# chenzpstar/Multi-Modal-Image-Fusion

Measured on AMD Instinct MI355X. Metric: image-pairs/sec at 256x256, PFNet train step, higher is better.
Workload: dtype bf16; 1 GPU; PFNetv1 train step (fwd + SSIM/pixel/grad losses + bwd + clip + Adam), 256x256 synthetic IR/visible pairs, batch 32 per GPU, bf16 feature maps / fp32 accumulate, random-init weights (seed 0); global_batch=32, parallelism=single

## Files before the change

### include/mmif.h

```cpp
#ifndef MMIF_H
#define MMIF_H

#include <stddef.h>
#include <stdint.h>

#ifdef __cplusplus
extern "C" {
#endif

#define MMIF_F32 0
#define MMIF_BF16 1

#define MMIF_IMPL_AUTO 0
#define MMIF_IMPL_VALU 1
#define MMIF_IMPL_MFMA 2
#define MMIF_IMPL_X3 3

#define MMIF_OK 0
#define MMIF_EINVAL (-1)
#define MMIF_ELAUNCH (-2)
#define MMIF_EWORKSPACE (-3)

typedef struct mmif_tensor {
    void* data;
// ... 242 lines not shown
size_t mmif_fusion_loss_workspace(int32_t n, int32_t h, int32_t w);
int mmif_fusion_loss(const float* img1, const float* img2, const float* imgf, int32_t n, int32_t h, int32_t w, float w_ssim,
                     float data_range, float w_pixel, int32_t pixel_max, int32_t pixel_l2, float w_grad, int32_t grad_max,
                     int32_t grad_l2, float* loss_out, float* grad_out, void* workspace, size_t workspace_bytes, void* stream);

int mmif_conv2d_bwd_pair_supported(int32_t cin, int32_t cout, int32_t ksize);
int mmif_conv2d_reflect_bwd_pair(const mmif_tensor* gy, const void* w_packed_t, const mmif_tensor* x, const mmif_tensor* gx, float* dw, float* db,
                                 int32_t cin, int32_t cout, int32_t ksize, int32_t accumulate, void* workspace, size_t workspace_bytes,
                                 void* stream);

int mmif_conv2d_bwd_wide_supported(int32_t cin, int32_t cout, int32_t ksize);
int mmif_conv2d_bwd_wide_supported_f32(int32_t cin, int32_t cout, int32_t ksize);
size_t mmif_conv2d_bwd_wide_signs_bytes(int32_t n, int32_t cin, int32_t h, int32_t w);
int mmif_conv2d_reflect_bwd_wide(const mmif_tensor* gy, const void* w_packed_t, const mmif_tensor* x, const mmif_tensor* gx, float* dw, float* db,
                                 int32_t cin, int32_t cout, int32_t ksize, uint64_t mask_bits, int32_t accumulate, void* workspace,
                                 size_t workspace_bytes, void* signs, size_t signs_bytes, void* stream);

typedef struct mmif_dense_encoder {
    const float* img;
    const float* w0;
    const float* b0;
    const void* packed[3];
    const float* bias[3];
} mmif_dense_encoder;
int mmif_dense_encoder_fwd(const mmif_dense_encoder* enc_a, const mmif_tensor* out_a, const mmif_dense_encoder* enc_b,
                           const mmif_tensor* out_b, void* stream);
int32_t mmif_dense_encoder_fwd_sum_supported(const mmif_dense_encoder* enc_a, const mmif_dense_encoder* enc_b, int32_t n, int32_t h, int32_t w);
int mmif_dense_encoder_fwd_sum(const mmif_dense_encoder* enc_a, const mmif_tensor* out_a, const mmif_dense_encoder* enc_b,
                               const mmif_tensor* out_b, const mmif_tensor* sum, void* stream);

size_t mmif_dense_encoder_wgrad_workspace(void);
int mmif_dense_encoder_wgrad(const float* img, const mmif_tensor* x, const mmif_tensor* gz, float* dw0, float* db0, float* dw1, float* db1,
                             float* dw2, float* db2, float* dw3, float* db3, int32_t accumulate, void* workspace, size_t workspace_bytes,
                             void* stream);

int mmif_pack_dense_chain(const float* w1, const float* w2, const float* w3, void* packed_v0, void* packed_v1, void* packed_v2,
                          void* stream);
int mmif_pack_dense_chain_pair(const float* const* w_a, void* const* packed_a, const float* const* w_b, void* const* packed_b, void* stream);
typedef struct mmif_dense_chain {
    const mmif_tensor* g3;
    const mmif_tensor* glow;
    const mmif_tensor* x;
    const void* packed[3];
    const mmif_tensor* out;
} mmif_dense_chain;
int mmif_dense_encoder_chain(const mmif_dense_chain* chain_a, const mmif_dense_chain* chain_b, void* stream);
int32_t mmif_dense_encoder_bwd_fits(int32_t cb_total, int32_t h, int32_t w, int32_t halo);
size_t mmif_dense_encoder_bwd_workspace(void);
int mmif_dense_encoder_bwd(const mmif_dense_chain* chain_a, const float* img_a, float* const* dwdb_a, int32_t accumulate_a,
                           const mmif_dense_chain* chain_b, const float* img_b, float* const* dwdb_b, int32_t accumulate_b,
                           void* workspace, size_t workspace_bytes, void* stream);
int mmif_pack_dense_chain_x3(const float* w1, const float* w2, const float* w3, void* packed_v0, void* packed_v1, void* packed_v2,
                             void* stream);

int mmif_patch_feed(const uint8_t* bank, int64_t n_patches, int32_t patch, const int32_t* idx, const int32_t* mode, int32_t batch,
                    int32_t norm_mode, float* out, void* stream);

size_t mmif_clip_adam_workspace(int64_t numel);
int mmif_clip_adam_step(float* params, const float* grads, float* exp_avg, float* exp_avg_sq, int64_t numel,
                        float lr, float beta1, float beta2, float eps, int32_t step, float max_norm,
                        float grad_scale, float* norm_out, void* workspace, size_t workspace_bytes, void* stream);

void mmif_debug_set_trace(void* device_buf);
void mmif_debug_set_conv_dma(int32_t mode);
void mmif_debug_set_conv1x1_stream(int32_t mode);
void mmif_debug_set_bwd_pair_dma(int32_t mode);
void mmif_debug_set_thin_wide(int32_t mode);
void mmif_debug_set_wgrad_dma_blocks(int32_t blocks);
void mmif_debug_set_ragged(int32_t mode);
int mmif_reduce_defer_begin(void* arena, size_t bytes);
int mmif_reduce_defer_flush(int32_t keep_deferring, void* stream);
int32_t mmif_reduce_defer_pending(void);

enum { MMIF_ROUTE_FWD = 0, MMIF_ROUTE_DGRAD = 1, MMIF_ROUTE_DGRAD_ONTO = 2, MMIF_ROUTE_DGRAD_DUP = 3, MMIF_ROUTE_WGRAD = 4, MMIF_ROUTE_BWD_PAIR = 5,
       MMIF_ROUTE_BWD_WIDE = 6 };
typedef struct {
    char name[32];
    int32_t G, slices, tiles, org;
} mmif_route;
int mmif_conv2d_route(int32_t op, const mmif_tensor* a, const mmif_tensor* b, int32_t cin, int32_t cout, int32_t ksize, uint64_t mask_bits,
                      uint64_t accum_bits, int32_t fold, int32_t impl, int32_t num_cus, mmif_route* out);

void mmif_debug_set_enc_stream2(int32_t mode);

#ifdef __cplusplus
}
#endif
#endif
```

### multi-modal-image-fusion_amd/csrc/loss.hip

```cpp
#include <math.h>

#include "common.hpp"

namespace mmif {

struct Win11 {
    float t[11];
};

constexpr int LT = 16;
constexpr int WIN = 11;

constexpr int ST = 32;
constexpr int SIN = ST + WIN - 1;
constexpr int SPI = 44;
constexpr int SPH = 36;

typedef float lf32x2 __attribute__((ext_vector_type(2)));

__device__ inline void ld16(const float* p, float (&v)[16]) {
#pragma unroll
    for (int i = 0; i < 4; ++i) {
        const float4 q = *reinterpret_cast<const float4*>(p + 4 * i);
        v[4 * i] = q.x; v[4 * i + 1] = q.y; v[4 * i + 2] = q.z; v[4 * i + 3] = q.w;
    }
}

__global__ __launch_bounds__(256, 2) void ssim_stats_kernel(const float* __restrict__ x1, const float* __restrict__ x2,
                                                            const float* __restrict__ f, int H, int W, Win11 win, float C1,
                                                            float C2, float* __restrict__ maps ,
                                                            float* __restrict__ partial, int tiles_x) {
    __shared__ __attribute__((aligned(16))) float in[3][SIN][SPI];
    __shared__ __attribute__((aligned(16))) float hb[8][SIN][SPH];
    __shared__ float red[16];
    const int Hm = H - WIN + 1, Wm = W - WIN + 1;
    const int tid = threadIdx.x;
    const int mx0 = (blockIdx.x % tiles_x) * ST, my0 = (blockIdx.x / tiles_x) * ST;
    const int in_ = blockIdx.y;
    const long long ibase = (long long)in_ * H * W;
    for (int e = tid; e < SIN * SPI; e += 256) {
        const int py = e / SPI, px = e % SPI;
        const int y = my0 + py, x = mx0 + px;
        const bool ok = (y < H) && (x < W) && px < SIN;
        const long long i = ibase + (long long)min(y, H - 1) * W + min(x, W - 1);
        const float a = x1[i], b = x2[i], c = f[i];
        in[0][py][px] = ok ? a : 0.f;
        in[1][py][px] = ok ? b : 0.f;
        in[2][py][px] = ok ? c : 0.f;
    }
    __syncthreads();
#pragma unroll 1
    for (int r = 0; r < 3; ++r) {
        const int it = tid + 256 * r, set = it / 384, idx = it - set * 384;
        if (idx >= SIN * 8) continue;
        const int py = idx >> 3, cg = idx & 7;
        float xa[16], fc[16];
        ld16(&in[set][py][4 * cg], xa);
        ld16(&in[2][py][4 * cg], fc);
        lf32x2 pa[14], pc[14];
#pragma unroll
        for (int i = 0; i < 14; ++i) {
            const float a = xa[i], c = fc[i];
            pa[i] = (lf32x2){a, a * a};
            pc[i] = (lf32x2){a * c, set ? c * c : c};
        }
        lf32x2 s01[4], s23[4];
#pragma unroll
        for (int j = 0; j < 4; ++j) s01[j] = s23[j] = (lf32x2){0.f, 0.f};
#pragma unroll
        for (int k = 0; k < WIN; ++k) {
            const lf32x2 wk = (lf32x2){win.t[k], win.t[k]};
#pragma unroll
            for (int j = 0; j < 4; ++j) {
                s01[j] = __builtin_elementwise_fma(wk, pa[j + k], s01[j]);
                s23[j] = __builtin_elementwise_fma(wk, pc[j + k], s23[j]);
            }
        }
        const int q0 = set ? 1 : 0, q1 = set ? 4 : 3, q2 = set ? 7 : 6, q3 = set ? 5 : 2;
        *reinterpret_cast<float4*>(&hb[q0][py][4 * cg]) = make_float4(s01[0].x, s01[1].x, s01[2].x, s01[3].x);
        *reinterpret_cast<float4*>(&hb[q1][py][4 * cg]) = make_float4(s01[0].y, s01[1].y, s01[2].y, s01[3].y);
        *reinterpret_cast<float4*>(&hb[q2][py][4 * cg]) = make_float4(s23[0].x, s23[1].x, s23[2].x, s23[3].x);
        *reinterpret_cast<float4*>(&hb[q3][py][4 * cg]) = make_float4(s23[0].y, s23[1].y, s23[2].y, s23[3].y);
    }
    __syncthreads();
    const int tx = tid & 31, rg = tid >> 5;
    float m[8][4];
#pragma unroll
    for (int q = 0; q < 8; q += 2) {
        lf32x2 v[14];
#pragma unroll
        for (int i = 0; i < 14; ++i) v[i] = (lf32x2){hb[q][4 * rg + i][tx], hb[q + 1][4 * rg + i][tx]};
#pragma unroll
        for (int j = 0; j < 4; ++j) {
            lf32x2 acc = (lf32x2){0.f, 0.f};
#pragma unroll
            for (int k = 0; k < WIN; ++k) acc = __builtin_elementwise_fma((lf32x2){win.t[k], win.t[k]}, v[j + k], acc);
            m[q][j] = acc.x;
            m[q + 1][j] = acc.y;
        }
    }
    float ssum = 0.f;
    const long long msz = (long long)gridDim.y * Hm * Wm;
#pragma unroll
    for (int j = 0; j < 4; ++j) {
        const int my = my0 + 4 * rg + j, mx = mx0 + tx;
        if (!((my < Hm) && (mx < Wm))) continue;
        const float mu1 = m[0][j], mu2 = m[1][j], muf = m[2][j];
        const float sf_raw = m[5][j] - muf * muf;
        const float sf = fmaxf(sf_raw, 0.f);
        const float kf = sf_raw > 0.f ? 1.f : 0.f;
        float A = 0.f, B = 0.f, Cs[2];
#pragma unroll
        for (int s2 = 0; s2 < 2; ++s2) {
            const float mux = s2 == 0 ? mu1 : mu2;
            const float ex2 = s2 == 0 ? m[3][j] : m[4][j];
            const float exf = s2 == 0 ? m[6][j] : m[7][j];
            const float sx = fmaxf(ex2 - mux * mux, 0.f);
            const float sxf = exf - mux * muf;
            const float m1 = 2.f * mux * muf + C1, m2 = mux * mux + muf * muf + C1;
            const float v1 = 2.f * sxf + C2, v2 = sx + sf + C2;
            const float inv = 1.f / (m2 * v2);
            const float S = m1 * v1 * inv;
            ssum += S;
            const float Bp = -(S / v2) * kf;
            const float Cp = 2.f * m1 * inv;
            const float Ap = 2.f * mux * v1 * inv - 2.f * muf * S / m2 - 2.f * mux * m1 * inv - 2.f * muf * Bp;
            A += Ap;
            B += Bp;
            Cs[s2] = Cp;
        }
        if (maps != nullptr) {
            const long long mi = ((long long)in_ * Hm + my) * Wm + mx;
            maps[mi] = A;
            maps[msz + mi] = B;
            maps[2 * msz + mi] = Cs[0];
            maps[3 * msz + mi] = Cs[1];
        }
    }
    const float bs = block_sum(ssum, red);
    if (tid == 0) partial[(long long)in_ * gridDim.x + blockIdx.x] = bs;
}

__global__ __launch_bounds__(256, 2) void ssim_grad_kernel(const float* __restrict__ x1, const float* __restrict__ x2,
                                                           const float* __restrict__ f, int H, int W, Win11 win,
                                                           const float* __restrict__ maps, float scale,
                                                           float* __restrict__ grad, int tiles_x) {
    __shared__ __attribute__((aligned(16))) float in[4][SIN][SPI];
    __shared__ __attribute__((aligned(16))) float hb[4][SIN][SPH];
    const int Hm = H - WIN + 1, Wm = W - WIN + 1;
    const int tid = threadIdx.x;
    const int x0 = (blockIdx.x % tiles_x) * ST, y0 = (blockIdx.x / tiles_x) * ST;
    const int in_ = blockIdx.y;
    const long long msz = (long long)gridDim.y * Hm * Wm;
    for (int e = tid; e < SIN * SPI; e += 256) {
        const int py = e / SPI, px = e % SPI;
        const int my = y0 - (WIN - 1) + py, mx = x0 - (WIN - 1) + px;
        const bool ok = my >= 0 && my < Hm && mx >= 0 && mx < Wm && px < SIN;
        const long long mi = ((long long)in_ * Hm + min(max(my, 0), Hm - 1)) * Wm + min(max(mx, 0), Wm - 1);
#pragma unroll
        for (int q = 0; q < 4; ++q) {
            const float v = maps[q * msz + mi];
            in[q][py][px] = ok ? v : 0.f;
        }
    }
    __syncthreads();
#pragma unroll 1
    for (int r = 0; r < 2; ++r) {
        const int idx = tid + 256 * r;
        if (idx >= SIN * 8) continue;
        const int py = idx >> 3, cg = idx & 7;
#pragma unroll
        for (int q = 0; q < 4; q += 2) {
            float v0[16], v1[16];
            ld16(&in[q][py][4 * cg], v0);
            ld16(&in[q + 1][py][4 * cg], v1);
            lf32x2 v[14];
#pragma unroll
            for (int i = 0; i < 14; ++i) v[i] = (lf32x2){v0[i], v1[i]};
            lf32x2 s2[4];
#pragma unroll
            for (int j = 0; j < 4; ++j) s2[j] = (lf32x2){0.f, 0.f};
#pragma unroll
            for (int k = 0; k < WIN; ++k)
#pragma unroll
                for (int j = 0; j < 4; ++j) s2[j] = __builtin_elementwise_fma((lf32x2){win.t[k], win.t[k]}, v[j + (WIN - 1) - k], s2[j]);
            *reinterpret_cast<float4*>(&hb[q][py][4 * cg]) = make_float4(s2[0].x, s2[1].x, s2[2].x, s2[3].x);
            *reinterpret_cast<float4*>(&hb[q + 1][py][4 * cg]) = make_float4(s2[0].y, s2[1].y, s2[2].y, s2[3].y);
        }
    }
    __syncthreads();
    const int tx = tid & 31, rg = tid >> 5;
    float m[4][4];
#pragma unroll
    for (int q = 0; q < 4; q += 2) {
        lf32x2 v[14];
#pragma unroll
        for (int i = 0; i < 14; ++i) v[i] = (lf32x2){hb[q][4 * rg + i][tx], hb[q + 1][4 * rg + i][tx]};
#pragma unroll
        for (int j = 0; j < 4; ++j) {
            lf32x2 acc = (lf32x2){0.f, 0.f};
#pragma unroll
            for (int k = 0; k < WIN; ++k) acc = __builtin_elementwise_fma((lf32x2){win.t[k], win.t[k]}, v[j + (WIN - 1) - k], acc);
            m[q][j] = acc.x;
            m[q + 1][j] = acc.y;
        }
    }
#pragma unroll
    for (int j = 0; j < 4; ++j) {
        const int y = y0 + 4 * rg + j, x = x0 + tx;
        if (y < H && x < W) {
            const long long i = ((long long)in_ * H + y) * W + x;
            grad[i] = scale * (m[0][j] + 2.f * f[i] * m[1][j] + x1[i] * m[2][j] + x2[i] * m[3][j]);
        }
    }
}

__global__ void ssim_finish_kernel(const float* __restrict__ partial, int np, float weight, float inv_count,
                                   float* __restrict__ loss) {
    __shared__ float red[16];
    float s = 0.f;
    for (int i = threadIdx.x; i < np; i += blockDim.x) s += partial[i];
    const float t = block_sum(s, red);
    if (threadIdx.x == 0) loss[0] = weight * (1.f - 0.5f * t * inv_count);
}

__global__ __launch_bounds__(256) void pixel_loss_kernel(const float* __restrict__ x1, const float* __restrict__ x2,
                                                         const float* __restrict__ f, long long total, float gscale,
                                                         int mode_max, int l2, float* __restrict__ grad,
                                                         float* __restrict__ partial, int accum) {
    __shared__ float red[16];
    float s = 0.f;
    for (long long i = (long long)blockIdx.x * blockDim.x + threadIdx.x; i < total; i += (long long)gridDim.x * blockDim.x) {
        const float a = x1[i], b = x2[i], c = f[i];
        float g;
        if (mode_max) {
            const float d = c - fmaxf(a, b);
            s += l2 ? d * d : fabsf(d);
            g = l2 ? 2.f * d : (d > 0.f ? 1.f : (d < 0.f ? -1.f : 0.f));
        } else {
            const float d1 = c - a, d2 = c - b;
            s += 0.5f * (l2 ? d1 * d1 + d2 * d2 : fabsf(d1) + fabsf(d2));
            g = 0.5f * (l2 ? 2.f * (d1 + d2)
                           : ((d1 > 0.f ? 1.f : (d1 < 0.f ? -1.f : 0.f)) + (d2 > 0.f ? 1.f : (d2 < 0.f ? -1.f : 0.f))));
        }
        if (grad) grad[i] = accum ? grad[i] + gscale * g : gscale * g;
    }
    const float t = block_sum(s, red);
    if (threadIdx.x == 0) partial[blockIdx.x] = t;
}

__global__ void scale_finish_kernel(const float* __restrict__ partial, int np, float scale, float* __restrict__ loss) {
    __shared__ float red[16];
    float s = 0.f;
    for (int i = threadIdx.x; i < np; i += blockDim.x) s += partial[i];
    const float t = block_sum(s, red);
    if (threadIdx.x == 0) loss[0] = scale * t;
}

constexpr int FF_CAP = 12288;
__device__ inline float ff_ordered_sum(const float* __restrict__ p, int n, float* lds) {
    const bool staged = n <= FF_CAP;
    __syncthreads();
    if (staged)
        for (int i = threadIdx.x; i < n; i += blockDim.x) lds[i] = p[i];
    __syncthreads();
    float s = 0.f;
    if (threadIdx.x < 256) {
        if (staged) for (int i = threadIdx.x; i < n; i += 256) s += lds[i];
        else for (int i = threadIdx.x; i < n; i += 256) s += p[i];
    }
    return s;
}
__global__ __launch_bounds__(1024) void fusion_finish_kernel(const float* __restrict__ ps, int ns, float w_ssim, float inv_count,
                                                             const float* __restrict__ pp, int npx, float scale_px, const float* __restrict__ pg,
                                                             int ngr, float scale_gr, float* __restrict__ out) {
    __shared__ float red[16];
    __shared__ float stage[FF_CAP];
    const float ta = block_sum(ff_ordered_sum(ps, ns, stage), red);
    const float tb = block_sum(ff_ordered_sum(pp, npx, stage), red);
    const float tc = block_sum(ff_ordered_sum(pg, ngr, stage), red);
    if (threadIdx.x == 0) {
        const float l1 = w_ssim * (1.f - 0.5f * ta * inv_count), l2 = scale_px * tb, l3 = scale_gr * tc;
        out[0] = (l1 + l2) + l3;
        out[1] = l1; out[2] = l2; out[3] = l3;
        out[4] = out[0];
    }
}

constexpr int GH = 3;
constexpr int GIN = LT + 2 * GH;
constexpr int DH = 2;
constexpr int GD = LT + 2 * DH;

__device__ inline float sgnf(float v) { return v > 0.f ? 1.f : (v < 0.f ? -1.f : 0.f); }

__global__ __launch_bounds__(256) void grad_loss_kernel(const float* __restrict__ x1, const float* __restrict__ x2,
                                                        const float* __restrict__ f, int H, int W, float gscale,
                                                        int mode_max, int l2, float* __restrict__ grad,
                                                        float* __restrict__ partial, int tiles_x, int accum,
                                                        int px_mode = -1, float gscale_px = 0.f, float* __restrict__ part_px = nullptr) {
    __shared__ float in[3][GIN][52];
    __shared__ float dx[GD][48], dy[GD][48];
    __shared__ float red[16];
    const int tid = threadIdx.x, tx = tid & 15, ty = tid >> 4;
    const int x0 = (blockIdx.x % tiles_x) * LT, y0 = (blockIdx.x / tiles_x) * LT;
    const int in_ = blockIdx.y;
    const long long ibase = (long long)in_ * H * W;
    for (int e = tid; e < GIN * GIN; e += 256) {
        const int py = e / GIN, px = e % GIN;
        const int y = min(max(reflect_idx(y0 - GH + py, H), 0), H - 1);
        const int x = min(max(reflect_idx(x0 - GH + px, W), 0), W - 1);
        const long long i = ibase + (long long)y * W + x;
        in[0][py][px] = x1[i];
        in[1][py][px] = x2[i];
        in[2][py][px] = f[i];
    }
    __syncthreads();
    float lsum = 0.f;
    for (int e = tid; e < GD * GD; e += 256) {
        const int py = e / GD, px = e % GD;
        const int y = y0 - DH + py, x = x0 - DH + px;
        float vx = 0.f, vy = 0.f;
        if (y >= 0 && y < H && x >= 0 && x < W) {
            float mag[3], sx = 0.f, sy = 0.f;
#pragma unroll
            for (int q = 0; q < 3; ++q) {
                const int cy = py + GH - DH, cx = px + GH - DH;
                const float a00 = in[q][cy - 1][cx - 1], a01 = in[q][cy - 1][cx], a02 = in[q][cy - 1][cx + 1];
                const float a10 = in[q][cy][cx - 1], a12 = in[q][cy][cx + 1];
                const float a20 = in[q][cy + 1][cx - 1], a21 = in[q][cy + 1][cx], a22 = in[q][cy + 1][cx + 1];
                const float gx = (a02 - a00) + 2.f * (a12 - a10) + (a22 - a20);
                const float gy = (a20 - a00) + 2.f * (a21 - a01) + (a22 - a02);
                mag[q] = fabsf(gx) + fabsf(gy);
                if (q == 2) { sx = sgnf(gx); sy = sgnf(gy); }
            }
            float s, l;
            if (mode_max) {
                const float d = mag[2] - fmaxf(mag[0], mag[1]);
                l = l2 ? d * d : fabsf(d);
                s = l2 ? 2.f * d : sgnf(d);
            } else {
                const float d1 = mag[2] - mag[0], d2 = mag[2] - mag[1];
                l = 0.5f * (l2 ? d1 * d1 + d2 * d2 : fabsf(d1) + fabsf(d2));
                s = 0.5f * (l2 ? 2.f * (d1 + d2) : sgnf(d1) + sgnf(d2));
            }
            vx = s * sx;
            vy = s * sy;
            if (py >= DH && py < DH + LT && px >= DH && px < DH + LT) lsum += l;
        }
        dx[py][px] = vx;
        dy[py][px] = vy;
    }
    __syncthreads();
    const int y = y0 + ty, x = x0 + tx;
    if (grad != nullptr && y < H && x < W) {
        auto D = [&](int qy, int qx, bool isx) -> float {
            if (qy < 0 || qy >= H || qx < 0 || qx >= W) return 0.f;
            const int ly = qy - y0 + DH, lx = qx - x0 + DH;
            return isx ? dx[ly][lx] : dy[ly][lx];
        };
        auto Tq = [&](int qy, int qx) -> float {
            float t = 0.f;
            t += -1.f * D(qy + 1, qx + 1, true) + 1.f * D(qy + 1, qx - 1, true);
            t += -2.f * D(qy, qx + 1, true) + 2.f * D(qy, qx - 1, true);
            t += -1.f * D(qy - 1, qx + 1, true) + 1.f * D(qy - 1, qx - 1, true);
            t += -1.f * D(qy + 1, qx + 1, false) - 2.f * D(qy + 1, qx, false) - 1.f * D(qy + 1, qx - 1, false);
            t += 1.f * D(qy - 1, qx + 1, false) + 2.f * D(qy - 1, qx, false) + 1.f * D(qy - 1, qx - 1, false);
            return t;
        };
        int ys[3], xs[3], ny = 1, nx = 1;
        ys[0] = y;
        xs[0] = x;
        if (y == 1) ys[ny++] = -1;
        if (y == H - 2) ys[ny++] = H;
        if (x == 1) xs[nx++] = -1;
        if (x == W - 2) xs[nx++] = W;
        float g = 0.f;
        for (int a = 0; a < ny; ++a)
            for (int b = 0; b < nx; ++b) g += Tq(ys[a], xs[b]);
        float* gp = grad + ibase + (long long)y * W + x;
        float base = accum ? *gp : 0.f;
        if (px_mode >= 0) {
            const float a = in[0][ty + GH][tx + GH], b = in[1][ty + GH][tx + GH], c = in[2][ty + GH][tx + GH];
            float pg;
            if (px_mode & 1) {
                const float d = c - fmaxf(a, b);
                pg = (px_mode & 2) ? 2.f * d : sgnf(d);
            } else {
                const float d1 = c - a, d2 = c - b;
                pg = 0.5f * ((px_mode & 2) ? 2.f * (d1 + d2) : sgnf(d1) + sgnf(d2));
            }
            base = base + gscale_px * pg;
        }
        *gp = (accum || px_mode >= 0) ? base + gscale * g : gscale * g;
    }
    float psum = 0.f;
    if (px_mode >= 0 && y < H && x < W) {
        const float a = in[0][ty + GH][tx + GH], b = in[1][ty + GH][tx + GH], c = in[2][ty + GH][tx + GH];
        if (px_mode & 1) {
            const float d = c - fmaxf(a, b);
            psum = (px_mode & 2) ? d * d : fabsf(d);
        } else {
            const float d1 = c - a, d2 = c - b;
            psum = 0.5f * ((px_mode & 2) ? d1 * d1 + d2 * d2 : fabsf(d1) + fabsf(d2));
        }
    }
    const float t = block_sum(lsum, red);
    if (tid == 0) partial[(long long)in_ * gridDim.x + blockIdx.x] = t;
    if (px_mode >= 0) {
        __syncthreads();
        const float tp = block_sum(psum, red);
        if (tid == 0) part_px[(long long)in_ * gridDim.x + blockIdx.x] = tp;
    }
}

void gaussian_window(Win11& w) {
    float g[WIN];
    double sum = 0.0;
    for (int i = 0; i < WIN; ++i) {
        g[i] = (float)exp(-(double)((i - WIN / 2) * (i - WIN / 2)) / (2.0 * 1.5 * 1.5));
        sum += (double)g[i];
    }
    const float fs = (float)sum;
    for (int i = 0; i < WIN; ++i) w.t[i] = g[i] / fs;
}

}

using namespace mmif;

extern "C" size_t mmif_loss_workspace(int32_t n, int32_t h, int32_t w) {
    const size_t tiles = (size_t)cdiv(h, LT) * cdiv(w, LT) * n;
    const size_t maps = (size_t)4 * n * (h > 10 ? h - 10 : 0) * (w > 10 ? w - 10 : 0);
    return (tiles + 4096 + maps) * sizeof(float);
}

extern "C" int mmif_ssim_loss(const float* img1, const float* img2, const float* imgf, int32_t n, int32_t h, int32_t w,
                              float weight, float data_range, float* loss_out, float* grad_out, void* workspace,
                              size_t workspace_bytes, void* stream) {
    MMIF_REQUIRE(h >= WIN && w >= WIN, "ssim_loss: image smaller than the 11x11 window (%dx%d)", h, w);
    if (workspace_bytes < mmif_loss_workspace(n, h, w)) {
        set_error("ssim_loss: workspace too small");
        return MMIF_EWORKSPACE;
    }
    hipStream_t st = (hipStream_t)stream;
    Win11 win;
    gaussian_window(win);
    const float C1 = (0.01f * data_range) * (0.01f * data_range), C2 = (0.03f * data_range) * (0.03f * data_range);
    const int Hm = h - WIN + 1, Wm = w - WIN + 1;
    const int tmx = cdiv(Wm, ST), tmy = cdiv(Hm, ST);
    float* partial = (float*)workspace;
    const int np = tmx * tmy * n;
    float* maps = grad_out ? partial + (((size_t)np + 63) / 64) * 64 : nullptr;
    hipLaunchKernelGGL(ssim_stats_kernel, dim3(tmx * tmy, n), dim3(256), 0, st, img1, img2, imgf, h, w, win, C1, C2, maps,
                       partial, tmx);
    if (int rc = check_launch("ssim_stats")) return rc;
    hipLaunchKernelGGL(ssim_finish_kernel, dim3(1), dim3(256), 0, st, partial, np, weight, 1.f / ((float)n * Hm * Wm),
                       loss_out);
    if (int rc = check_launch("ssim_finish")) return rc;
    if (grad_out) {
        const int tx = cdiv(w, ST), ty = cdiv(h, ST);
        const float scale = -weight * 0.5f / ((float)n * Hm * Wm);
        hipLaunchKernelGGL(ssim_grad_kernel, dim3(tx * ty, n), dim3(256), 0, st, img1, img2, imgf, h, w, win, maps, scale,
                           grad_out, tx);
        if (int rc = check_launch("ssim_grad")) return rc;
    }
    return MMIF_OK;
}

extern "C" int mmif_pixel_loss(const float* img1, const float* img2, const float* imgf, int32_t n, int32_t h, int32_t w,
                               float weight, int32_t mode_max, int32_t l2, float* loss_out, float* grad_out,
                               void* workspace, size_t workspace_bytes, void* stream) {
    if (workspace_bytes < mmif_loss_workspace(n, h, w)) {
        set_error("pixel_loss: workspace too small");
        return MMIF_EWORKSPACE;
    }
    hipStream_t st = (hipStream_t)stream;
    const long long total = (long long)n * h * w;
    int nb = cdiv(total, 256);
    if (nb > 2048) nb = 2048;
    float* partial = (float*)workspace;
    hipLaunchKernelGGL(pixel_loss_kernel, dim3(nb), dim3(256), 0, st, img1, img2, imgf, total, weight / (float)total, mode_max,
                       l2, grad_out, partial, 0);
    if (int rc = check_launch("pixel_loss")) return rc;
    hipLaunchKernelGGL(scale_finish_kernel, dim3(1), dim3(256), 0, st, partial, nb, weight / (float)total, loss_out);
    return check_launch("pixel_finish");
}

extern "C" int mmif_grad_loss(const float* img1, const float* img2, const float* imgf, int32_t n, int32_t h, int32_t w,
                              float weight, int32_t mode_max, int32_t l2, float* loss_out, float* grad_out,
                              void* workspace, size_t workspace_bytes, void* stream) {
    MMIF_REQUIRE(h >= 2 && w >= 2, "grad_loss: reflect padding needs h,w >= 2");
    if (workspace_bytes < mmif_loss_workspace(n, h, w)) {
        set_error("grad_loss: workspace too small");
        return MMIF_EWORKSPACE;
    }
    hipStream_t st = (hipStream_t)stream;
    const int tx = cdiv(w, LT), ty = cdiv(h, LT);
    const long long total = (long long)n * h * w;
    float* partial = (float*)workspace;
    hipLaunchKernelGGL(grad_loss_kernel, dim3(tx * ty, n), dim3(256), 0, st, img1, img2, imgf, h, w, weight / (float)total,
                       mode_max, l2, grad_out, partial, tx, 0);
    if (int rc = check_launch("grad_loss")) return rc;
    hipLaunchKernelGGL(scale_finish_kernel, dim3(1), dim3(256), 0, st, partial, tx * ty * n, weight / (float)total, loss_out);
    return check_launch("grad_finish");
}

static size_t fusion_parts(int32_t n, int32_t h, int32_t w, size_t* o_px, size_t* o_gr, size_t* o_maps) {
    const int Hm = h - WIN + 1, Wm = w - WIN + 1;
    const size_t ns = (size_t)cdiv(Wm, ST) * cdiv(Hm, ST) * n, ngr = (size_t)cdiv(w, LT) * cdiv(h, LT) * n;
    auto up = [](size_t v) { return (v + 63) / 64 * 64; };
    *o_px = up(ns);
    *o_gr = *o_px + up(ngr);
    *o_maps = *o_gr + up(ngr);
    return *o_maps + (size_t)4 * n * (h > 10 ? h - 10 : 0) * (w > 10 ? w - 10 : 0);
}
extern "C" size_t mmif_fusion_loss_workspace(int32_t n, int32_t h, int32_t w) {
    size_t a, b, c;
    return fusion_parts(n, h, w, &a, &b, &c) * sizeof(float);
}
extern "C" int mmif_fusion_loss(const float* img1, const float* img2, const float* imgf, int32_t n, int32_t h, int32_t w, float w_ssim,
                                float data_range, float w_pixel, int32_t pixel_max, int32_t pixel_l2, float w_grad, int32_t grad_max,
                                int32_t grad_l2, float* loss_out, float* grad_out, void* workspace, size_t workspace_bytes, void* stream) {
    MMIF_REQUIRE(h >= WIN && w >= WIN, "fusion_loss: image smaller than the 11x11 window (%dx%d)", h, w);
    size_t o_px, o_gr, o_maps;
    if (workspace_bytes < fusion_parts(n, h, w, &o_px, &o_gr, &o_maps) * sizeof(float)) {
        set_error("fusion_loss: workspace too small");
        return MMIF_EWORKSPACE;
    }
    hipStream_t st = (hipStream_t)stream;
    Win11 win;
    gaussian_window(win);
    const float C1 = (0.01f * data_range) * (0.01f * data_range), C2 = (0.03f * data_range) * (0.03f * data_range);
    const int Hm = h - WIN + 1, Wm = w - WIN + 1;
    const int tmx = cdiv(Wm, ST), tmy = cdiv(Hm, ST);
    float* ps = (float*)workspace;
    float *pp = ps + o_px, *pg = ps + o_gr, *maps = grad_out ? ps + o_maps : nullptr;
    const int ns = tmx * tmy * n;
    hipLaunchKernelGGL(ssim_stats_kernel, dim3(tmx * tmy, n), dim3(256), 0, st, img1, img2, imgf, h, w, win, C1, C2, maps, ps, tmx);
    if (int rc = check_launch("fusion_loss ssim_stats")) return rc;
    if (grad_out) {
        const int tx = cdiv(w, ST), ty = cdiv(h, ST);
        hipLaunchKernelGGL(ssim_grad_kernel, dim3(tx * ty, n), dim3(256), 0, st, img1, img2, imgf, h, w, win, maps,
                           -w_ssim * 0.5f / ((float)n * Hm * Wm), grad_out, tx);
        if (int rc = check_launch("fusion_loss ssim_grad")) return rc;
    }
    const long long total = (long long)n * h * w;
    const int tx = cdiv(w, LT), ty = cdiv(h, LT);
    hipLaunchKernelGGL(grad_loss_kernel, dim3(tx * ty, n), dim3(256), 0, st, img1, img2, imgf, h, w, w_grad / (float)total, grad_max, grad_l2,
                       grad_out, pg, tx, 1, (pixel_max ? 1 : 0) | (pixel_l2 ? 2 : 0), w_pixel / (float)total, pp);
    if (int rc = check_launch("fusion_loss pixel + grad")) return rc;
    hipLaunchKernelGGL(fusion_finish_kernel, dim3(1), dim3(1024), 0, st, ps, ns, w_ssim, 1.f / ((float)n * Hm * Wm), pp, tx * ty * n,
                       w_pixel / (float)total, pg, tx * ty * n, w_grad / (float)total, loss_out);
    return check_launch("fusion_loss finish");
}
```

### multi-modal-image-fusion_amd/mmif/_lib.py

```python
import ctypes as C
import os

import torch

_HERE = os.path.dirname(os.path.abspath(__file__))
LIB_PATH = os.environ.get("MMIF_LIB") or os.path.join(os.path.dirname(_HERE), "libmmif_hip.so")

F32, BF16 = 0, 1
IMPL_AUTO, IMPL_VALU, IMPL_MFMA, IMPL_X3 = 0, 1, 2, 3
PACK_BF16, PACK_X3 = 0, 1
FUSE_SUM, FUSE_MEAN, FUSE_MAX = 0, 1, 2
T_FOLDED = 1


class MmifTensor(C.Structure):
    _fields_ = [("data", C.c_void_p), ("dtype", C.c_int32), ("n", C.c_int32), ("h", C.c_int32), ("w", C.c_int32),
                ("halo", C.c_int32), ("cb_total", C.c_int32), ("cb_off", C.c_int32), ("cb", C.c_int32), ("flags", C.c_int32)]


class MmifPackJob(C.Structure):
    _fields_ = [("w", C.c_void_p), ("cout", C.c_int32), ("cin", C.c_int32), ("ksize", C.c_int32), ("format", C.c_int32),
                ("packed_fwd", C.c_void_p), ("packed_dgrad", C.c_void_p)]


# ... 101 lines not shown
    "mmif_dense_encoder_bwd": (_i32, [C.POINTER(MmifDenseChain), _vp, C.POINTER(C.c_void_p), _i32, C.POINTER(MmifDenseChain), _vp, C.POINTER(C.c_void_p), _i32,
                                      _vp, _sz, _vp]),
    "mmif_dense_encoder_wgrad_workspace": (_sz, []),
    "mmif_dense_encoder_wgrad": (_i32, [_vp, _TP, _TP] + [_vp] * 8 + [_i32, _vp, _sz, _vp]),
    "mmif_act_fwd": (_i32, [_vp, _vp, _i64, _i32, _f32, _vp]),
    "mmif_act_bwd": (_i32, [_vp, _vp, _vp, _i64, _i32, _f32, _vp]),
    "mmif_conv2d_reflect_fwd": (_i32, [_TP, _vp, _vp, _vp, _TP, _i32, _i32, _i32, _i32, _i32, _vp]),
    "mmif_conv2d_reflect_dgrad": (_i32, [_TP, _vp, _vp, _TP, _TP, _i32, _i32, _i32, _u64, _u64, _i32, _vp]),
    "mmif_conv2d_dgrad_onto_supported": (_i32, [_TP, _TP, _i32, _i32, _i32]),
    "mmif_conv2d_reflect_dgrad_folded_onto": (_i32, [_TP, _vp, _TP, _TP, _TP, _i32, _i32, _i32, _u64, _u64, _vp]),
    "mmif_conv2d_reflect_dgrad_folded": (_i32, [_TP, _vp, _vp, _TP, _TP, _i32, _i32, _i32, _u64, _u64, _i32, _vp]),
    "mmif_conv2d_route": (_i32, [_i32, _TP, _TP, _i32, _i32, _i32, _u64, _u64, _i32, _i32, _i32, C.POINTER(MmifRoute)]),
    "mmif_conv2d_wgrad_workspace": (_sz, [_i32, _i32, _i32]),
    "mmif_conv2d_reflect_wgrad": (_i32, [_TP, _TP, _vp, _vp, _i32, _i32, _i32, _i32, _vp, _sz, _i32, _vp]),
    "mmif_conv2d_image_in_fwd": (_i32, [_vp, _vp, _vp, _TP, _i32, _i32, _i32, _vp]),
    "mmif_conv2d_image_in_wgrad": (_i32, [_vp, _TP, _vp, _vp, _i32, _i32, _i32, _vp, _sz, _vp]),
    "mmif_conv2d_image_out_fwd": (_i32, [_TP, _vp, _vp, _vp, _i32, _i32, _i32, _vp]),
    "mmif_conv2d_image_out_dgrad": (_i32, [_vp, _vp, _vp, _TP, _TP, _i32, _i32, _u64, _u64, _vp]),
    "mmif_conv2d_image_out_wgrad": (_i32, [_TP, _vp, _vp, _vp, _vp, _i32, _i32, _i32, _vp, _sz, _vp]),
    "mmif_conv2d_image_wgrad_workspace": (_sz, [_i32, _i32]),
    "mmif_conv2d_image_out_bwd_supported": (_i32, [_i32, _i32, _i32, _i32, _i32]),
    "mmif_conv2d_image_out_bwd": (_i32, [_TP, _vp, _vp, _vp, _TP, _vp, _vp, _i32, _i32, _i32, _vp, _sz, _vp]),
    "mmif_fuse_elem_fwd": (_i32, [_TP, _TP, _TP, _i32, _vp]),
    "mmif_fuse_elem_bwd": (_i32, [_TP, _TP, _TP, _TP, _TP, _i32, _i32, _vp]),
    "mmif_fuse_attn_workspace": (_sz, [_i32, _i32]),
    "mmif_fuse_attn_fwd": (_i32, [_TP, _TP, _TP, _i32, _vp, _sz, _vp]),
    "mmif_fuse_attn_bwd": (_i32, [_TP, _TP, _TP, _TP, _TP, _i32, _i32, _vp, _sz, _vp]),
    "mmif_fuse_attn_bwd_cached": (_i32, [_TP, _TP, _TP, _TP, _TP, _i32, _i32, _vp, _sz, _vp]),
    "mmif_nonlocal_spatial_workspace": (_sz, [_i32] * 4),
    "mmif_nonlocal_spatial_fwd": (_i32, [_vp] * 4 + [_i32] * 4 + [_vp, _sz, _vp]),
    "mmif_nonlocal_spatial_bwd": (_i32, [_vp] * 6 + [_i32] * 4 + [_vp, _sz, _vp]),
    "mmif_sra_workspace": (_sz, [_i32, _i32, _i32, _i64, _i64]),
    "mmif_sra_fwd": (_i32, [_vp] * 5 + [_i32, _i32, _i32, _i64, _i64, _f32, _vp]),
    "mmif_sra_bwd": (_i32, [_vp] * 9 + [_i32, _i32, _i32, _i64, _i64, _f32, _vp, _sz, _vp]),
    "mmif_layernorm_fwd": (_i32, [_vp] * 5 + [_i32, _i32, _i64, _f32, _vp]),
    "mmif_glue_workspace": (_sz, [_i32]),
    "mmif_layernorm_bwd": (_i32, [_vp] * 7 + [_i32, _i32, _i64, _vp, _sz, _vp]),
    "mmif_join_fwd": (_i32, [_vp] * 5 + [_i32, _i32, _i64, _i32, _vp]),
    "mmif_join_bwd": (_i32, [_vp] * 10 + [_i32, _i32, _i64, _i32, _vp, _sz, _vp]),
    "mmif_pairconv_fwd": (_i32, [_TP, _TP, _vp, _vp, _i32, _TP, _TP, _i32, _TP, _TP, _vp]),
    "mmif_pairconv_dgrad": (_i32, [_TP, _TP, _vp, _i32, _TP, _TP, _TP, _TP, _u64, _TP, _vp]),
    "mmif_pairconv_wgrad_workspace": (_sz, []),
    "mmif_pairconv_wgrad": (_i32, [_TP, _TP, _TP, _TP, _i32, _vp, _vp, _i32, _vp, _sz, _vp]),
    "mmif_pairconv_bwd": (_i32, [_TP, _TP, _vp, _i32, _TP, _TP, _TP, _TP, _u64, _TP, _vp, _vp, _i32, _vp, _sz, _vp]),
    "mmif_maxpool2x2_fwd": (_i32, [_TP, _TP, _vp]),
    "mmif_maxpool2x2_bwd": (_i32, [_TP, _TP, _TP, _i32, _vp]),
    "mmif_upsample2x_fwd": (_i32, [_TP, _TP, _vp]),
    "mmif_upsample2x_bwd": (_i32, [_TP, _TP, _i32, _vp]),
    "mmif_relu_mask": (_i32, [_TP, _TP, _vp]),
    "mmif_maxpool2x2_bwd_relu": (_i32, [_TP, _TP, _TP, _i32, _vp]),
    "mmif_upsample2x_bwd_relu": (_i32, [_TP, _TP, _i32, _TP, _vp]),
    "mmif_loss_workspace": (_sz, [_i32, _i32, _i32]),
    "mmif_ssim_loss": (_i32, [_vp, _vp, _vp, _i32, _i32, _i32, _f32, _f32, _vp, _vp, _vp, _sz, _vp]),
    "mmif_ssim_loss_mode_workspace": (_sz, [_i32, _i32, _i32, _i32]),
    "mmif_ssim_loss_mode": (_i32, [_vp, _vp, _vp, _i32, _i32, _i32, _f32, _f32, _i32, _vp, _vp, _vp, _sz, _vp]),
    "mmif_ssim_terms": (_i32, [_vp, _vp, _i32, _i32, _i32, _i32, _f32, _vp, _vp, _sz, _vp]),
    "mmif_metric_moments_workspace": (_sz, [_i32] * 4),
    "mmif_metric_moments": (_i32, [_vp, _i32, _i32, _i32, _i32, _vp, _vp, _sz, _vp]),
    "mmif_metric_hist": (_i32, [_vp, _vp, _i32, _i32, _i32, _vp, _vp, _vp, _vp]),
    "mmif_metric_entropy": (_i32, [_vp, _vp, _vp, _i32, _i64, _vp, _vp]),
    "mmif_metric_qabf_workspace": (_sz, [_i32] * 3),
    "mmif_metric_qabf": (_i32, [_vp, _vp, _vp, _i32, _i32, _i32, _f64, _vp, _vp, _sz, _vp]),
    "mmif_metric_vif_workspace": (_sz, [_i32] * 3),
    "mmif_metric_vif": (_i32, [_vp, _vp, _vp, _i32, _i32, _i32, _vp, _vp, _vp, _sz, _vp]),
    "mmif_metric_msssim_workspace": (_sz, [_i32] * 3),
    "mmif_metric_msssim": (_i32, [_vp, _vp, _vp, _i32, _i32, _i32, _f32, _vp, _vp, _sz, _vp]),
    "mmif_tv_loss_workspace": (_sz, []),
    "mmif_tv_loss": (_i32, [_vp, _i32, _i32, _i32, _f32, _i32, _vp, _vp, _vp, _sz, _vp]),
    "mmif_pixel_loss": (_i32, [_vp, _vp, _vp, _i32, _i32, _i32, _f32, _i32, _i32, _vp, _vp, _vp, _sz, _vp]),
    "mmif_grad_loss": (_i32, [_vp, _vp, _vp, _i32, _i32, _i32, _f32, _i32, _i32, _vp, _vp, _vp, _sz, _vp]),
    "mmif_fusion_loss_workspace": (_sz, [_i32, _i32, _i32]),
    "mmif_fusion_loss": (_i32, [_vp, _vp, _vp, _i32, _i32, _i32, _f32, _f32, _f32, _i32, _i32, _f32, _i32, _i32, _vp, _vp, _vp, _sz, _vp]),
    "mmif_patch_feed": (_i32, [_vp, _i64, _i32, _vp, _vp, _i32, _i32, _vp, _vp]),
    "mmif_clip_adam_workspace": (_sz, [_i64]),
    "mmif_clip_adam_step": (_i32, [_vp, _vp, _vp, _vp, _i64, _f32, _f32, _f32, _f32, _i32, _f32, _f32, _vp, _vp, _sz, _vp]),
    "mmif_debug_set_trace": (None, [_vp]),
    "mmif_debug_set_conv_dma": (None, [_i32]),
    "mmif_debug_set_conv1x1_stream": (None, [_i32]),
    "mmif_debug_set_bwd_pair_dma": (None, [_i32]),
    "mmif_debug_set_thin_wide": (None, [_i32]),
    "mmif_debug_set_wgrad_dma_blocks": (None, [_i32]),
    "mmif_debug_set_ragged": (None, [_i32]),
    "mmif_debug_set_enc_stream2": (None, [_i32]),
    "mmif_probe_tr16": (_i32, [_vp, _vp, _vp]),
    "mmif_probe_mfma": (_i32, [_vp, _vp, _vp, _vp]),
    "mmif_probe_dma": (_i32, [_vp, _vp, _vp, _vp, _vp]),
}

for _name, (_res, _args) in SIGNATURES.items():
    _fn = getattr(lib, _name)
    _fn.restype = _res
    _fn.argtypes = _args


def check(rc, what=""):
    if rc != 0:
        raise MmifError(f"{what or 'mmif'} failed (code {rc}): {lib.mmif_last_error().decode()}")


def version():
    return lib.mmif_version().decode()
```

Baseline: 9095 image-pairs/s.

## Fuse loss finish and pixel/grad accumulation into SSIM grad kernel; halve stats LDS

The pixel+gradient loss kernel now runs first and writes its gradient into a separate workspace plane. The SSIM gradient kernel then adds that plane plus the pixel term in its epilogue, and one block also computes the final loss reduction, so the separate finish launch and the read-modify-write accumulate pass go away. The SSIM stats kernel processes its two image sets in turn through half-sized shared memory and asks for three blocks per SM instead of two. The cost is an extra full-size plane write and read, a serial finish inside block 0 of the grad kernel, and an added sync in the stats kernel.

```diff
diff --git a/include/mmif.h b/include/mmif.h
--- a/include/mmif.h
+++ b/include/mmif.h
@@ -348,6 +348,7 @@
                       uint64_t accum_bits, int32_t fold, int32_t impl, int32_t num_cus, mmif_route* out);
 
 void mmif_debug_set_enc_stream2(int32_t mode);
+void mmif_debug_set_loss_fork(int32_t mode);
 
 #ifdef __cplusplus
 }
diff --git a/multi-modal-image-fusion_amd/csrc/loss.hip b/multi-modal-image-fusion_amd/csrc/loss.hip
--- a/multi-modal-image-fusion_amd/csrc/loss.hip
+++ b/multi-modal-image-fusion_amd/csrc/loss.hip
@@ -26,12 +26,12 @@
     }
 }
 
-__global__ __launch_bounds__(256, 2) void ssim_stats_kernel(const float* __restrict__ x1, const float* __restrict__ x2,
+__global__ __launch_bounds__(256, 3) void ssim_stats_kernel(const float* __restrict__ x1, const float* __restrict__ x2,
                                                             const float* __restrict__ f, int H, int W, Win11 win, float C1,
                                                             float C2, float* __restrict__ maps ,
                                                             float* __restrict__ partial, int tiles_x) {
     __shared__ __attribute__((aligned(16))) float in[3][SIN][SPI];
-    __shared__ __attribute__((aligned(16))) float hb[8][SIN][SPH];
+    __shared__ __attribute__((aligned(16))) float hb[4][SIN][SPH];
     __shared__ float red[16];
     const int Hm = H - WIN + 1, Wm = W - WIN + 1;
     const int tid = threadIdx.x;
@@ -49,54 +49,56 @@
         in[2][py][px] = ok ? c : 0.f;
     }
     __syncthreads();
-#pragma unroll 1
-    for (int r = 0; r < 3; ++r) {
-        const int it = tid + 256 * r, set = it / 384, idx = it - set * 384;
-        if (idx >= SIN * 8) continue;
-        const int py = idx >> 3, cg = idx & 7;
-        float xa[16], fc[16];
-        ld16(&in[set][py][4 * cg], xa);
-        ld16(&in[2][py][4 * cg], fc);
-        lf32x2 pa[14], pc[14];
-#pragma unroll
-        for (int i = 0; i < 14; ++i) {
-            const float a = xa[i], c = fc[i];
-            pa[i] = (lf32x2){a, a * a};
-            pc[i] = (lf32x2){a * c, set ? c * c : c};
-        }
-        lf32x2 s01[4], s23[4];
-#pragma unroll
-        for (int j = 0; j < 4; ++j) s01[j] = s23[j] = (lf32x2){0.f, 0.f};
-#pragma unroll
-        for (int k = 0; k < WIN; ++k) {
-            const lf32x2 wk = (lf32x2){win.t[k], win.t[k]};
-#pragma unroll
-            for (int j = 0; j < 4; ++j) {
-                s01[j] = __builtin_elementwise_fma(wk, pa[j + k], s01[j]);
-                s23[j] = __builtin_elementwise_fma(wk, pc[j + k], s23[j]);
-            }
-        }
-        const int q0 = set ? 1 : 0, q1 = set ? 4 : 3, q2 = set ? 7 : 6, q3 = set ? 5 : 2;
-        *reinterpret_cast<float4*>(&hb[q0][py][4 * cg]) = make_float4(s01[0].x, s01[1].x, s01[2].x, s01[3].x);
-        *reinterpret_cast<float4*>(&hb[q1][py][4 * cg]) = make_float4(s01[0].y, s01[1].y, s01[2].y, s01[3].y);
-        *reinterpret_cast<float4*>(&hb[q2][py][4 * cg]) = make_float4(s23[0].x, s23[1].x, s23[2].x, s23[3].x);
-        *reinterpret_cast<float4*>(&hb[q3][py][4 * cg]) = make_float4(s23[0].y, s23[1].y, s23[2].y, s23[3].y);
-    }
-    __syncthreads();
     const int tx = tid & 31, rg = tid >> 5;
     float m[8][4];
 #pragma unroll
-    for (int q = 0; q < 8; q += 2) {
-        lf32x2 v[14];
-#pragma unroll
-        for (int i = 0; i < 14; ++i) v[i] = (lf32x2){hb[q][4 * rg + i][tx], hb[q + 1][4 * rg + i][tx]};
-#pragma unroll
-        for (int j = 0; j < 4; ++j) {
-            lf32x2 acc = (lf32x2){0.f, 0.f};
-#pragma unroll
-            for (int k = 0; k < WIN; ++k) acc = __builtin_elementwise_fma((lf32x2){win.t[k], win.t[k]}, v[j + k], acc);
-            m[q][j] = acc.x;
-            m[q + 1][j] = acc.y;
+    for (int set = 0; set < 2; ++set) {
+        if (set) __syncthreads();
+#pragma unroll 1
+        for (int idx = tid; idx < SIN * 8; idx += 256) {
+            const int py = idx >> 3, cg = idx & 7;
+            float xa[16], fc[16];
+            ld16(&in[set][py][4 * cg], xa);
+            ld16(&in[2][py][4 * cg], fc);
+            lf32x2 pa[14], pc[14];
+#pragma unroll
+            for (int i = 0; i < 14; ++i) {
+                const float a = xa[i], c = fc[i];
+                pa[i] = (lf32x2){a, a * a};
+                pc[i] = (lf32x2){a * c, set ? c * c : c};
+            }
+            lf32x2 s01[4], s23[4];
+#pragma unroll
+            for (int j = 0; j < 4; ++j) s01[j] = s23[j] = (lf32x2){0.f, 0.f};
+#pragma unroll
+            for (int k = 0; k < WIN; ++k) {
+                const lf32x2 wk = (lf32x2){win.t[k], win.t[k]};
+#pragma unroll
+                for (int j = 0; j < 4; ++j) {
+                    s01[j] = __builtin_elementwise_fma(wk, pa[j + k], s01[j]);
+                    s23[j] = __builtin_elementwise_fma(wk, pc[j + k], s23[j]);
+                }
+            }
+            *reinterpret_cast<float4*>(&hb[0][py][4 * cg]) = make_float4(s01[0].x, s01[1].x, s01[2].x, s01[3].x);
+            *reinterpret_cast<float4*>(&hb[1][py][4 * cg]) = make_float4(s01[0].y, s01[1].y, s01[2].y, s01[3].y);
+            *reinterpret_cast<float4*>(&hb[2][py][4 * cg]) = make_float4(s23[0].x, s23[1].x, s23[2].x, s23[3].x);
+            *reinterpret_cast<float4*>(&hb[3][py][4 * cg]) = make_float4(s23[0].y, s23[1].y, s23[2].y, s23[3].y);
+        }
+        __syncthreads();
+        auto qs = [set](int p) { return set ? (p == 0 ? 1 : p == 1 ? 4 : p == 2 ? 7 : 5) : (p == 0 ? 0 : p == 1 ? 3 : p == 2 ? 6 : 2); };
+#pragma unroll
+        for (int p = 0; p < 4; p += 2) {
+            lf32x2 v[14];
+#pragma unroll
+            for (int i = 0; i < 14; ++i) v[i] = (lf32x2){hb[p][4 * rg + i][tx], hb[p + 1][4 * rg + i][tx]};
+#pragma unroll
+            for (int j = 0; j < 4; ++j) {
+                lf32x2 acc = (lf32x2){0.f, 0.f};
+#pragma unroll
+                for (int k = 0; k < WIN; ++k) acc = __builtin_elementwise_fma((lf32x2){win.t[k], win.t[k]}, v[j + k], acc);
+                m[qs(p)][j] = acc.x;
+                m[qs(p + 1)][j] = acc.y;
+            }
         }
     }
     float ssum = 0.f;
@@ -141,12 +143,69 @@
     if (tid == 0) partial[(long long)in_ * gridDim.x + blockIdx.x] = bs;
 }
 
+constexpr int FF_CAP = 12288;
+__device__ inline float ff_ordered_sum(const float* __restrict__ p, int n, float* lds) {
+    const bool staged = lds != nullptr && n <= FF_CAP;
+    __syncthreads();
+    if (staged)
+        for (int i = threadIdx.x; i < n; i += blockDim.x) lds[i] = p[i];
+    __syncthreads();
+    float s = 0.f;
+    if (threadIdx.x < 256) {
+        if (staged) for (int i = threadIdx.x; i < n; i += 256) s += lds[i];
+        else {
+#pragma unroll 16
+            for (int i = threadIdx.x; i < n; i += 256) s += p[i];
+        }
+    }
+    return s;
+}
+struct FusionFinish {
+    const float *ps, *pp, *pg;
+    int ns, npx, ngr;
+    float w_ssim, inv_count, scale_px, scale_gr;
+    float* out;
+};
+__device__ inline void fusion_finish_block(const FusionFinish& a, float* stage, float* red) {
+    const float ta = block_sum(ff_ordered_sum(a.ps, a.ns, stage), red);
+    const float tb = block_sum(ff_ordered_sum(a.pp, a.npx, stage), red);
+    const float tc = block_sum(ff_ordered_sum(a.pg, a.ngr, stage), red);
+    if (threadIdx.x == 0) {
+        const float l1 = a.w_ssim * (1.f - 0.5f * ta * a.inv_count), l2 = a.scale_px * tb, l3 = a.scale_gr * tc;
+        a.out[0] = (l1 + l2) + l3;
+        a.out[1] = l1; a.out[2] = l2; a.out[3] = l3;
+        a.out[4] = a.out[0];
+    }
+}
+__global__ __launch_bounds__(1024) void fusion_finish_kernel(FusionFinish a) {
+    __shared__ float red[16];
+    __shared__ float stage[FF_CAP];
+    fusion_finish_block(a, stage, red);
+}
+
+__device__ inline float sgnf(float v) { return v > 0.f ? 1.f : (v < 0.f ? -1.f : 0.f); }
+
+__device__ inline float pixel_grad_term(float a, float b, float c, int px_mode) {
+    if (px_mode & 1) {
+        const float d = c - fmaxf(a, b);
+        return (px_mode & 2) ? 2.f * d : sgnf(d);
+    }
+    const float d1 = c - a, d2 = c - b;
+    return 0.5f * ((px_mode & 2) ? 2.f * (d1 + d2) : sgnf(d1) + sgnf(d2));
+}
+
 __global__ __launch_bounds__(256, 2) void ssim_grad_kernel(const float* __restrict__ x1, const float* __restrict__ x2,
                                                            const float* __restrict__ f, int H, int W, Win11 win,
                                                            const float* __restrict__ maps, float scale,
-                                                           float* __restrict__ grad, int tiles_x) {
+                                                           float* __restrict__ grad, int tiles_x,
+                                                           const float* __restrict__ gplane = nullptr, float gscale = 0.f,
+                                                           float gscale_px = 0.f, int px_mode = 0, FusionFinish fin = FusionFinish()) {
     __shared__ __attribute__((aligned(16))) float in[4][SIN][SPI];
     __shared__ __attribute__((aligned(16))) float hb[4][SIN][SPH];
+    if (fin.out != nullptr && blockIdx.x == 0 && blockIdx.y == 0) {
+        fusion_finish_block(fin, nullptr, &hb[0][0][0]);
+        __syncthreads();
+    }
     const int Hm = H - WIN + 1, Wm = W - WIN + 1;
     const int tid = threadIdx.x;
     const int x0 = (blockIdx.x % tiles_x) * ST, y0 = (blockIdx.x / tiles_x) * ST;
@@ -210,7 +269,13 @@
         const int y = y0 + 4 * rg + j, x = x0 + tx;
         if (y < H && x < W) {
             const long long i = ((long long)in_ * H + y) * W + x;
-            grad[i] = scale * (m[0][j] + 2.f * f[i] * m[1][j] + x1[i] * m[2][j] + x2[i] * m[3][j]);
+            const float a = x1[i], b = x2[i], c = f[i];
+            float sg = scale * (m[0][j] + 2.f * c * m[1][j] + a * m[2][j] + b * m[3][j]);
+            if (gplane != nullptr) {
+                asm volatile("" : "+v"(sg));
+                sg = __builtin_fmaf(gscale, gplane[i], __builtin_fmaf(gscale_px, pixel_grad_term(a, b, c, px_mode), sg));
+            }
+            grad[i] = sg;
         }
     }
 }
@@ -257,42 +322,10 @@
     if (threadIdx.x == 0) loss[0] = scale * t;
 }
 
-constexpr int FF_CAP = 12288;
-__device__ inline float ff_ordered_sum(const float* __restrict__ p, int n, float* lds) {
-    const bool staged = n <= FF_CAP;
-    __syncthreads();
-    if (staged)
-        for (int i = threadIdx.x; i < n; i += blockDim.x) lds[i] = p[i];
-    __syncthreads();
-    float s = 0.f;
-    if (threadIdx.x < 256) {
-        if (staged) for (int i = threadIdx.x; i < n; i += 256) s += lds[i];
-        else for (int i = threadIdx.x; i < n; i += 256) s += p[i];
-    }
-    return s;
-}
-__global__ __launch_bounds__(1024) void fusion_finish_kernel(const float* __restrict__ ps, int ns, float w_ssim, float inv_count,
-                                                             const float* __restrict__ pp, int npx, float scale_px, const float* __restrict__ pg,
-                                                             int ngr, float scale_gr, float* __restrict__ out) {
-    __shared__ float red[16];
-    __shared__ float stage[FF_CAP];
-    const float ta = block_sum(ff_ordered_sum(ps, ns, stage), red);
-    const float tb = block_sum(ff_ordered_sum(pp, npx, stage), red);
-    const float tc = block_sum(ff_ordered_sum(pg, ngr, stage), red);
-    if (threadIdx.x == 0) {
-        const float l1 = w_ssim * (1.f - 0.5f * ta * inv_count), l2 = scale_px * tb, l3 = scale_gr * tc;
-        out[0] = (l1 + l2) + l3;
-        out[1] = l1; out[2] = l2; out[3] = l3;
-        out[4] = out[0];
-    }
-}
-
 constexpr int GH = 3;
 constexpr int GIN = LT + 2 * GH;
 constexpr int DH = 2;
 constexpr int GD = LT + 2 * DH;
-
-__device__ inline float sgnf(float v) { return v > 0.f ? 1.f : (v < 0.f ? -1.f : 0.f); }
 
 __global__ __launch_bounds__(256) void grad_loss_kernel(const float* __restrict__ x1, const float* __restrict__ x2,
                                                         const float* __restrict__ f, int H, int W, float gscale,
@@ -379,20 +412,16 @@
         for (int a = 0; a < ny; ++a)
             for (int b = 0; b < nx; ++b) g += Tq(ys[a], xs[b]);
         float* gp = grad + ibase + (long long)y * W + x;
-        float base = accum ? *gp : 0.f;
-        if (px_mode >= 0) {
-            const float a = in[0][ty + GH][tx + GH], b = in[1][ty + GH][tx + GH], c = in[2][ty + GH][tx + GH];
-            float pg;
-            if (px_mode & 1) {
-                const float d = c - fmaxf(a, b);
-                pg = (px_mode & 2) ? 2.f * d : sgnf(d);
-            } else {
-                const float d1 = c - a, d2 = c - b;
-                pg = 0.5f * ((px_mode & 2) ? 2.f * (d1 + d2) : sgnf(d1) + sgnf(d2));
+        if (accum == 2) {
+            *gp = g;
+        } else {
+            float base = accum ? *gp : 0.f;
+            if (px_mode >= 0) {
+                const float pg = pixel_grad_term(in[0][ty + GH][tx + GH], in[1][ty + GH][tx + GH], in[2][ty + GH][tx + GH], px_mode);
+                base = base + gscale_px * pg;
             }
-            base = base + gscale_px * pg;
-        }
-        *gp = (accum || px_mode >= 0) ? base + gscale * g : gscale * g;
+            *gp = (accum || px_mode >= 0) ? base + gscale * g : gscale * g;
+        }
     }
     float psum = 0.f;
     if (px_mode >= 0 && y < H && x < W) {
@@ -506,25 +535,32 @@
     return check_launch("grad_finish");
 }
 
-static size_t fusion_parts(int32_t n, int32_t h, int32_t w, size_t* o_px, size_t* o_gr, size_t* o_maps) {
+static int g_loss_fork = [] {
+    const char* e = getenv("MMIF_LOSS_FORK");
+    return (e != nullptr && e[0] == '0') ? 0 : 1;
+}();
+extern "C" void mmif_debug_set_loss_fork(int32_t mode) { g_loss_fork = mode ? 1 : 0; }
+
+static size_t fusion_parts(int32_t n, int32_t h, int32_t w, size_t* o_px, size_t* o_gr, size_t* o_maps, size_t* o_plane) {
     const int Hm = h - WIN + 1, Wm = w - WIN + 1;
     const size_t ns = (size_t)cdiv(Wm, ST) * cdiv(Hm, ST) * n, ngr = (size_t)cdiv(w, LT) * cdiv(h, LT) * n;
     auto up = [](size_t v) { return (v + 63) / 64 * 64; };
     *o_px = up(ns);
     *o_gr = *o_px + up(ngr);
     *o_maps = *o_gr + up(ngr);
-    return *o_maps + (size_t)4 * n * (h > 10 ? h - 10 : 0) * (w > 10 ? w - 10 : 0);
+    *o_plane = up(*o_maps + (size_t)4 * n * (h > 10 ? h - 10 : 0) * (w > 10 ? w - 10 : 0));
+    return *o_plane + (size_t)n * h * w;
 }
 extern "C" size_t mmif_fusion_loss_workspace(int32_t n, int32_t h, int32_t w) {
-    size_t a, b, c;
-    return fusion_parts(n, h, w, &a, &b, &c) * sizeof(float);
+    size_t a, b, c, d;
+    return fusion_parts(n, h, w, &a, &b, &c, &d) * sizeof(float);
 }
 extern "C" int mmif_fusion_loss(const float* img1, const float* img2, const float* imgf, int32_t n, int32_t h, int32_t w, float w_ssim,
                                 float data_range, float w_pixel, int32_t pixel_max, int32_t pixel_l2, float w_grad, int32_t grad_max,
                                 int32_t grad_l2, float* loss_out, float* grad_out, void* workspace, size_t workspace_bytes, void* stream) {
     MMIF_REQUIRE(h >= WIN && w >= WIN, "fusion_loss: image smaller than the 11x11 window (%dx%d)", h, w);
-    size_t o_px, o_gr, o_maps;
-    if (workspace_bytes < fusion_parts(n, h, w, &o_px, &o_gr, &o_maps) * sizeof(float)) {
+    size_t o_px, o_gr, o_maps, o_plane;
+    if (workspace_bytes < fusion_parts(n, h, w, &o_px, &o_gr, &o_maps, &o_plane) * sizeof(float)) {
         set_error("fusion_loss: workspace too small");
         return MMIF_EWORKSPACE;
     }
@@ -537,20 +573,35 @@
     float* ps = (float*)workspace;
     float *pp = ps + o_px, *pg = ps + o_gr, *maps = grad_out ? ps + o_maps : nullptr;
     const int ns = tmx * tmy * n;
+    const long long total = (long long)n * h * w;
+    const int tx = cdiv(w, LT), ty = cdiv(h, LT);
+    const int sx = cdiv(w, ST), sy = cdiv(h, ST);
+    const int px_mode = (pixel_max ? 1 : 0) | (pixel_l2 ? 2 : 0);
+    const float gscale = w_grad / (float)total, gscale_px = w_pixel / (float)total, sscale = -w_ssim * 0.5f / ((float)n * Hm * Wm);
+    FusionFinish fin;
+    fin.ps = ps; fin.pp = pp; fin.pg = pg;
+    fin.ns = ns; fin.npx = tx * ty * n; fin.ngr = tx * ty * n;
+    fin.w_ssim = w_ssim; fin.inv_count = 1.f / ((float)n * Hm * Wm); fin.scale_px = gscale_px; fin.scale_gr = gscale;
+    fin.out = loss_out;
+
     hipLaunchKernelGGL(ssim_stats_kernel, dim3(tmx * tmy, n), dim3(256), 0, st, img1, img2, imgf, h, w, win, C1, C2, maps, ps, tmx);
     if (int rc = check_launch("fusion_loss ssim_stats")) return rc;
+    if (grad_out != nullptr && g_loss_fork != 0) {
+        float* plane = ps + o_plane;
+        hipLaunchKernelGGL(grad_loss_kernel, dim3(tx * ty, n), dim3(256), 0, st, img1, img2, imgf, h, w, gscale, grad_max, grad_l2, plane, pg, tx, 2,
+                           px_mode, gscale_px, pp);
+        if (int rc = check_launch("fusion_loss pixel + grad")) return rc;
+        hipLaunchKernelGGL(ssim_grad_kernel, dim3(sx * sy, n), dim3(256), 0, st, img1, img2, imgf, h, w, win, maps, sscale, grad_out, sx, plane, gscale,
+                           gscale_px, px_mode, fin);
+        return check_launch("fusion_loss ssim_grad (sum + finish)");
+    }
     if (grad_out) {
-        const int tx = cdiv(w, ST), ty = cdiv(h, ST);
-        hipLaunchKernelGGL(ssim_grad_kernel, dim3(tx * ty, n), dim3(256), 0, st, img1, img2, imgf, h, w, win, maps,
-                           -w_ssim * 0.5f / ((float)n * Hm * Wm), grad_out, tx);
+        hipLaunchKernelGGL(ssim_grad_kernel, dim3(sx * sy, n), dim3(256), 0, st, img1, img2, imgf, h, w, win, maps, sscale, grad_out, sx);
         if (int rc = check_launch("fusion_loss ssim_grad")) return rc;
     }
-    const long long total = (long long)n * h * w;
-    const int tx = cdiv(w, LT), ty = cdiv(h, LT);
-    hipLaunchKernelGGL(grad_loss_kernel, dim3(tx * ty, n), dim3(256), 0, st, img1, img2, imgf, h, w, w_grad / (float)total, grad_max, grad_l2,
-                       grad_out, pg, tx, 1, (pixel_max ? 1 : 0) | (pixel_l2 ? 2 : 0), w_pixel / (float)total, pp);
+    hipLaunchKernelGGL(grad_loss_kernel, dim3(tx * ty, n), dim3(256), 0, st, img1, img2, imgf, h, w, gscale, grad_max, grad_l2, grad_out, pg, tx, 1,
+                       px_mode, gscale_px, pp);
     if (int rc = check_launch("fusion_loss pixel + grad")) return rc;
-    hipLaunchKernelGGL(fusion_finish_kernel, dim3(1), dim3(1024), 0, st, ps, ns, w_ssim, 1.f / ((float)n * Hm * Wm), pp, tx * ty * n,
-                       w_pixel / (float)total, pg, tx * ty * n, w_grad / (float)total, loss_out);
+    hipLaunchKernelGGL(fusion_finish_kernel, dim3(1), dim3(1024), 0, st, fin);
     return check_launch("fusion_loss finish");
 }
diff --git a/multi-modal-image-fusion_amd/mmif/_lib.py b/multi-modal-image-fusion_amd/mmif/_lib.py
--- a/multi-modal-image-fusion_amd/mmif/_lib.py
+++ b/multi-modal-image-fusion_amd/mmif/_lib.py
@@ -207,6 +207,7 @@
     "mmif_debug_set_wgrad_dma_blocks": (None, [_i32]),
     "mmif_debug_set_ragged": (None, [_i32]),
     "mmif_debug_set_enc_stream2": (None, [_i32]),
+    "mmif_debug_set_loss_fork": (None, [_i32]),
     "mmif_probe_tr16": (_i32, [_vp, _vp, _vp]),
     "mmif_probe_mfma": (_i32, [_vp, _vp, _vp, _vp]),
     "mmif_probe_dma": (_i32, [_vp, _vp, _vp, _vp, _vp]),
```

Result: no change. 9110 image-pairs/s, median of 4 (+0.2%).
